# Xingskcs/Distributed-TensorFlow-Examples

Hardware: AMD Instinct MI355X
Metric: images/sec (whole node), MNIST CNN sync all-reduce (higher is better)
Workload: dtype bf16; 1 GPU; model=mnist_cnn (conv5x5x32-pool-conv5x5x64-pool-fc1024-dropout-fc10, 3274634 params), global_batch=1024, parallelism=dp1, per_gpu_batch=1024, optimizer=adam (TF1), hip_graph=True, steps_per_graph=4, join_deferred=True, distinct_gpus=1, grad_allreduce=none (1 rank), ranks_seen_by_comm=1

## Files before the change

csrc/kernels/imgconv12_fused.hip:

```cpp
#include "imgconv.h"
#include "imgconv1_common.h"

namespace dtfe {

namespace {

using namespace c1;

constexpr int WAVES = 13, THREADS = 64 * WAVES;
constexpr int CS = 32, KH = 5, KW = 5, LWP = 20, PS = 48, N2 = 64, NT = N2 / 16;
constexpr int K2 = KH * KW * CS, NK = K2 / 32, KP = K2 + 16;
constexpr int PH = HI / 2;
constexpr int LH = PH + KH - 1;
constexpr int QH = PH / 2, Q2 = QH * QH;
constexpr int P1N = PH * PH * NCH;
constexpr int P2N = Q2 * N2;
constexpr int W_EL = N2 * KP, IMG_EL = LH * LWP * PS;
constexpr int STAGE_B = P2N * 3, COPIES_B = 8 * CSZ * 2;
constexpr int UNION_B = COPIES_B > STAGE_B ? COPIES_B : STAGE_B;
constexpr int P_B = PRW * PWD * 2;
constexpr int LDS_B = W_EL * 2 + IMG_EL * 2 + UNION_B + P_B;
static_assert(W_EL * 2 == 104448 && IMG_EL * 2 == 34560 && STAGE_B == 9408 && COPIES_B == 20608 && P_B == 3072,
              "LDS regions");
static_assert(LDS_B == 162688 && LDS_B <= 160 * 1024, "LDS budget");
static_assert(K2 % 32 == 0 && PS >= CS + NCH / 2, "a pixel's pad bytes hold its 32 argmax bytes");
static_assert((PH * PH + 15) / 16 == WAVES, "one conv2 row tile per wave");

struct Conv12Args {
  ImgConvArgs c1;
  const bf16* w2;
  const float* b2;
  bf16* p2;
  uint8_t* a2;
};

template <int B, int E, typename F>
__device__ __forceinline__ void static_for(F&& f) {
  if constexpr (B < E) {
    f(std::integral_constant<int, B>{});
    static_for<B + 1, E>(f);
  }
}

__device__ __forceinline__ int row_window(int m) {
  const int t = m >> 4, quad = (m >> 2) & 3;
  const int w = t * 4 + (quad == 0 ? 0 : quad == 1 ? 2 : quad == 2 ? 3 : 1);
  return w < Q2 ? w : -1;
}

__global__ __launch_bounds__(THREADS) void conv12_fwd_kernel(Conv12Args A) {
  extern __shared__ __attribute__((aligned(16))) bf16 lds[];
  bf16* wl = lds;
  bf16* img = wl + W_EL;
  bf16* C = img + IMG_EL;
  bf16* sy = C;
  uint8_t* sa = reinterpret_cast<uint8_t*>(sy + P2N);
  bf16* P = C + UNION_B / 2;
  const ImgConvArgs& a = A.c1;
  const int tid = threadIdx.x, lane = tid & 63, wid = __builtin_amdgcn_readfirstlane(tid >> 6), g = lane >> 4;

  for (int i = tid; i < IMG_EL / 8; i += THREADS) reinterpret_cast<u32x4_t*>(img)[i] = u32x4_t{0u, 0u, 0u, 0u};
  for (int i = tid; i < PRW * PWD / 8; i += THREADS) reinterpret_cast<u32x4_t*>(P)[i] = u32x4_t{0u, 0u, 0u, 0u};

  const int64_t gstep = *a.g_counter;
  for (int z = 0; z < a.nz; ++z)
    for (long i = (long)blockIdx.x * THREADS + tid; i < a.zlen[z]; i += (long)gridDim.x * THREADS) a.zptr[z][i] = 0u;

  uint32_t px = 0u;
  int32_t lab = 0;
  auto fetch = [&](long bb) {
    const long r = (long)(hash_u32(a.g_seed, (uint64_t)gstep * a.B + bb) % (uint32_t)a.g_rows);
    if (tid < XCH) px = *reinterpret_cast<const uint32_t*>(a.g_src + r * (HI * HI) + tid * 4);
    if (tid == 0) lab = a.g_labels_src[r];
  };
  long b = blockIdx.x;
  if (b < a.B) fetch(b);

  {
    constexpr int kc_row = KP / 8, total = N2 * kc_row;
    static_assert(total <= 8 * THREADS, "one pass");
    u32x4_t v[8];
    int off[8];
#pragma unroll
    for (int u = 0; u < 8; ++u) {
      const int i = tid + u * THREADS;
      const int n = i / kc_row, k = (i - n * kc_row) * 8;
      off[u] = i < total ? n * KP + k : -1;
      v[u] = u32x4_t{0u, 0u, 0u, 0u};
      if (i < total && k < K2) v[u] = *reinterpret_cast<const u32x4_t*>(A.w2 + (long)n * K2 + k);
    }
#pragma unroll
    for (int u = 0; u < 8; ++u)
      if (off[u] >= 0) *reinterpret_cast<u32x4_t*>(wl + off[u]) = v[u];
  }

  bf16x8_t bw[2][2];
  float bias1[2];
  load_conv1_weights(a.w, a.bias, lane, g, bw, bias1);

  const bf16* wlane = wl + (lane & 15) * KP + 8 * g;
  float bias2[NT];
#pragma unroll
  for (int n = 0; n < NT; ++n) bias2[n] = A.b2 ? A.b2[n * 16 + (lane & 15)] : 0.f;
  const bf16* abase;
  {
    const int m = wid * 16 + (lane & 15), w = row_window(m), q = m & 3;
    const int oy = 2 * (w / QH) + (q >> 1), ox = 2 * (w % QH) + (q & 1);
    abase = img + (w >= 0 ? (oy * LWP + ox) * PS : 0) + 8 * g;
  }
  const int ppix = row_window(wid * 16 + g * 4);

  __syncthreads();
  for (; b < a.B; b += gridDim.x) {
    if (tid < XCH) {
      const u32x2_t v = px4_to_bf16(px);
      *reinterpret_cast<u32x2_t*>(const_cast<bf16*>(a.src) + b * (HI * HI) + tid * 4) = v;
      write_img(P, v);
    }
    if (tid == 0 && a.g_labels_dst) a.g_labels_dst[b] = lab;
    __syncthreads();
    if (b + gridDim.x < a.B) fetch(b + gridDim.x);
    build_copies8_by4(P, C);
    __syncthreads();

    for (int t = wid; t < 49; t += WAVES) {
      const int m = t * 16 + (lane & 15), q = m & 3, w = m >> 2;
      const int oy = 2 * (w / 14) + (q >> 1), ox = 2 * (w % 14) + (q & 1);
      const int s = ox & 7;
      const bf16* ab = C + s * CSZ + (ox - s) + oy * CWD;
      const bf16x8_t a0 = __builtin_bit_cast(bf16x8_t, ld16l(ab + g * CWD));
      const bf16x8_t a1 = __builtin_bit_cast(bf16x8_t, ld16l(ab + 4 * CWD));
      f32x4_t acc[2];
#pragma unroll
      for (int nt = 0; nt < 2; ++nt) {
        acc[nt] = __builtin_amdgcn_mfma_f32_16x16x32_bf16(a0, bw[nt][0], f32x4_t{0.f, 0.f, 0.f, 0.f}, 0, 0, 0);
        acc[nt] = __builtin_amdgcn_mfma_f32_16x16x32_bf16(a1, bw[nt][1], acc[nt], 0, 0, 0);
      }
      const int wq = t * 4 + g, py = wq / 14, pxx = wq - py * 14;
      bf16* pp = img + ((py + 2) * LWP + pxx + 2) * PS;
      uint8_t* pa = reinterpret_cast<uint8_t*>(pp + CS);
#pragma unroll
      for (int nt = 0; nt < 2; ++nt) {
        const f32x4_t v = acc[nt];
        int am = 0;
        float mx = v[0];
#pragma unroll
        for (int j = 1; j < 4; ++j) if (v[j] > mx) { mx = v[j]; am = j; }
        const int ch = nt * 16 + (lane & 15);
        pp[ch] = f2bf(apply_act(mx + bias1[nt], ACT_RELU));
        pa[ch] = (uint8_t)am;
      }
    }
    __syncthreads();

    {
      const long ob = b * (long)P1N;
      for (int i = tid; i < P1N / 8 + P1N / 16; i += THREADS) {
        const bool isv = i < P1N / 8;
        const int k = isv ? i : i - P1N / 8;
        const int pix = isv ? k >> 2 : k >> 1, py = pix / PH, pxx = pix - py * PH;
        const bf16* pp = img + ((py + 2) * LWP + pxx + 2) * PS;
        if (isv) {
          *reinterpret_cast<u32x4_t*>(a.y + ob + k * 8) = *reinterpret_cast<const u32x4_t*>(pp + (k & 3) * 8);
        } else {
          *reinterpret_cast<u32x4_t*>(a.argmax + ob + k * 16) =
              *reinterpret_cast<const u32x4_t*>(reinterpret_cast<const uint8_t*>(pp + CS) + (k & 1) * 16);
        }
      }
    }

    f32x4_t acc[NT];
#pragma unroll
    for (int n = 0; n < NT; ++n) acc[n] = f32x4_t{0.f, 0.f, 0.f, 0.f};
    constexpr int PF = 2;
    u32x4_t fa[PF + 1], fb[PF + 1][NT];
    auto fetch_frag = [&](auto sc) {
      constexpr int st = decltype(sc)::value;
      constexpr int k0 = 32 * st, tap = k0 / CS, cs = k0 - tap * CS;
      constexpr int toff = ((tap / KW) * LWP + (tap % KW)) * PS + cs;
      constexpr int buf = st % (PF + 1);
      fa[buf] = *reinterpret_cast<const u32x4_t*>(abase + toff);
#pragma unroll
      for (int n = 0; n < NT; ++n) fb[buf][n] = *reinterpret_cast<const u32x4_t*>(wlane + n * 16 * KP + k0);
    };
    static_for<0, PF>([&](auto sc) { fetch_frag(sc); });
    static_for<0, NK>([&](auto sc) {
      constexpr int st = decltype(sc)::value;
      if constexpr (st + PF < NK) fetch_frag(std::integral_constant<int, st + PF>{});
      constexpr int buf = st % (PF + 1);
#pragma unroll
      for (int n = 0; n < NT; ++n)
        acc[n] = __builtin_amdgcn_mfma_f32_16x16x32_bf16(__builtin_bit_cast(bf16x8_t, fa[buf]),
                                                         __builtin_bit_cast(bf16x8_t, fb[buf][n]), acc[n], 0, 0, 0);
      constexpr int nm = NT, nr = (st + PF < NK) ? 1 + NT : 0;
      static_for<0, nm>([&](auto ic) {
        constexpr int i = decltype(ic)::value, r0 = i * nr / nm, r1 = (i + 1) * nr / nm;
        if constexpr (r1 > r0) __builtin_amdgcn_sched_group_barrier(0x100, r1 - r0, 0);
        __builtin_amdgcn_sched_group_barrier(0x8, 1, 0);
      });
    });
    if (ppix >= 0) {
#pragma unroll
      for (int n = 0; n < NT; ++n) {
        const int col = n * 16 + (lane & 15);
        const f32x4_t v = acc[n];
        int am = 0;
        float mx = v[0];
#pragma unroll
        for (int j = 1; j < 4; ++j) if (v[j] > mx) { mx = v[j]; am = j; }
        sy[ppix * N2 + col] = f2bf(apply_act(mx + bias2[n], ACT_RELU));
        sa[ppix * N2 + col] = (uint8_t)am;
      }
    }
    __syncthreads();
    {
      constexpr int ny = P2N / 8, na = P2N / 16;
      const long pb = b * (long)P2N;
      for (int i = tid; i < ny + na; i += THREADS) {
        if (i < ny) {
          *reinterpret_cast<u32x4_t*>(A.p2 + pb + i * 8) = *reinterpret_cast<const u32x4_t*>(sy + i * 8);
        } else {
          const int k = i - ny;
          *reinterpret_cast<u32x4_t*>(A.a2 + pb + k * 16) = *reinterpret_cast<const u32x4_t*>(sa + k * 16);
        }
      }
    }
  }
  if (a.g_done && tid == 0) {
    const uint32_t prev = __hip_atomic_fetch_add(a.g_done, 1u, __ATOMIC_RELAXED, __HIP_MEMORY_SCOPE_AGENT);
    if (prev == gridDim.x - 1) {
      __hip_atomic_fetch_add((unsigned long long*)a.g_counter, 1ull, __ATOMIC_RELAXED, __HIP_MEMORY_SCOPE_AGENT);
      __hip_atomic_store(a.g_done, 0u, __ATOMIC_RELAXED, __HIP_MEMORY_SCOPE_AGENT);
    }
  }
}

}

bool launch_conv12_fused_fwd(const ImgConvArgs& a, const bf16* w2, const float* b2, bf16* p2, uint8_t* a2,
                             hipStream_t s) {
  if (a.B < 256 || a.SH != HI || a.SW != HI || a.CS != 1 || a.OH != HI || a.OW != HI || a.N != NCH || a.KH != 5 ||
      a.KW != 5 || a.stride != 1 || a.pad != 2)
    return false;
  if (!a.src || !a.pool || a.flip_taps || a.dil > 1 || a.relu_mask || a.act != ACT_RELU) return false;
  if (!a.g_src || !a.g_counter || !a.g_labels_src || !a.y || !a.argmax || !w2 || !p2 || !a2) return false;
  Conv12Args A{a, w2, b2, p2, a2};
  A.c1.diag = 0;
  const int grid = a.B < 256 ? a.B : 256;
  (void)hipFuncSetAttribute((const void*)conv12_fwd_kernel, hipFuncAttributeMaxDynamicSharedMemorySize, LDS_B);
  hipLaunchKernelGGL(conv12_fwd_kernel, dim3(grid), dim3(THREADS), LDS_B, s, A);
  return true;
}

}
```

csrc/kernels/imgconv1_common.h:

```cpp
#pragma once
#include "common.h"

#include <type_traits>

namespace dtfe {
namespace c1 {

constexpr int TH = 256;
constexpr int HI = 28;
constexpr int PWD = 48, PRW = 32;
constexpr int CWD = 40;
constexpr int CSZ = PRW * CWD + 8;
constexpr int NCH = 32;
constexpr int XCH = HI * HI / 4;

__device__ __forceinline__ u32x4_t ld16l(const bf16* p) { return *reinterpret_cast<const u32x4_t*>(p); }

template <int B, int E, typename F>
__device__ __forceinline__ void static_for_c1(F&& f) {
  if constexpr (B < E) {
    f(std::integral_constant<int, B>{});
    static_for_c1<B + 1, E>(f);
  }
}

__device__ __forceinline__ void load_img(const bf16* x, long b, u32x2_t& v) {
  if (threadIdx.x < XCH) v = *reinterpret_cast<const u32x2_t*>(x + b * (HI * HI) + threadIdx.x * 4);
}
__device__ __forceinline__ void write_img(bf16* P, const u32x2_t& v) {
  if (threadIdx.x < XCH) {
    const int r = threadIdx.x / 7, c = (threadIdx.x - r * 7) * 4;
    *reinterpret_cast<u32x2_t*>(P + (r + 2) * PWD + c + 4) = v;
  }
}

__device__ __forceinline__ u32x2_t px4_to_bf16(uint32_t px) {
  const float k = 1.f / 255.f;
  return u32x2_t{pack_bf16x2((float)(px & 0xffu) * k, (float)((px >> 8) & 0xffu) * k),
                 pack_bf16x2((float)((px >> 16) & 0xffu) * k, (float)(px >> 24) * k)};
}

__device__ __forceinline__ uint32_t shr16(uint32_t lo, uint32_t hi) {
  return (uint32_t)((((uint64_t)hi << 32) | lo) >> 16);
}
template <int S>
__device__ __forceinline__ void build_copies(const bf16* P, bf16* C) {
  constexpr int HALF = (S + 1) / 2;
  const int t = threadIdx.x & 127, r = t >> 2, c8 = (t & 3) * 8;
  const u32x4_t* src = reinterpret_cast<const u32x4_t*>(P + r * PWD + c8);
  uint32_t d[12];
#pragma unroll
  for (int j = 0; j < 3; ++j) {
    const u32x4_t v = src[j];
#pragma unroll
    for (int e = 0; e < 4; ++e) d[4 * j + e] = v[e];
  }
  auto emit = [&](auto sc) {
    constexpr int s = decltype(sc)::value;
    constexpr int e0 = s + 2;
    u32x4_t o;
#pragma unroll
    for (int j = 0; j < 4; ++j) o[j] = (e0 & 1) ? shr16(d[(e0 >> 1) + j], d[(e0 >> 1) + j + 1]) : d[(e0 >> 1) + j];
    *reinterpret_cast<u32x4_t*>(C + s * CSZ + r * CWD + c8) = o;
  };
  if (threadIdx.x < 128) {
    static_for_c1<0, HALF>(emit);
  } else {
    static_for_c1<HALF, S>(emit);
  }
}

__device__ __forceinline__ void build_copies8_by4(const bf16* P, bf16* C) {
  if (threadIdx.x >= 512) return;
  const int t = threadIdx.x & 127, r = t >> 2, c8 = (t & 3) * 8;
  const u32x4_t* src = reinterpret_cast<const u32x4_t*>(P + r * PWD + c8);
  uint32_t d[12];
#pragma unroll
  for (int j = 0; j < 3; ++j) {
    const u32x4_t v = src[j];
#pragma unroll
    for (int e = 0; e < 4; ++e) d[4 * j + e] = v[e];
  }
  auto emit = [&](auto sc) {
    constexpr int s = decltype(sc)::value;
    constexpr int e0 = s + 2;
    u32x4_t o;
#pragma unroll
    for (int j = 0; j < 4; ++j) o[j] = (e0 & 1) ? shr16(d[(e0 >> 1) + j], d[(e0 >> 1) + j + 1]) : d[(e0 >> 1) + j];
    *reinterpret_cast<u32x4_t*>(C + s * CSZ + r * CWD + c8) = o;
  };
  switch (threadIdx.x >> 7) {
    case 0: static_for_c1<0, 2>(emit); break;
    case 1: static_for_c1<2, 4>(emit); break;
    case 2: static_for_c1<4, 6>(emit); break;
    default: static_for_c1<6, 8>(emit); break;
  }
}

__device__ __forceinline__ void load_conv1_weights(const bf16* w, const float* bias, int lane, int g,
                                                   bf16x8_t (&bw)[2][2], float (&biasv)[2]) {
#pragma unroll
  for (int nt = 0; nt < 2; ++nt) {
    const int n = nt * 16 + (lane & 15);
    biasv[nt] = bias ? bias[n] : 0.f;
#pragma unroll
    for (int st = 0; st < 2; ++st) {
      const int kh = st == 0 ? g : 4;
      const bool rowok = st == 0 || g == 0;
      s16x8_t v;
#pragma unroll
      for (int j = 0; j < 8; ++j) v[j] = (short)((rowok && j < 5) ? w[n * 25 + kh * 5 + j] : 0);
      bw[nt][st] = __builtin_bit_cast(bf16x8_t, v);
    }
  }
}

}
}
```

Before: 5.609 million images/sec.

## Add producer waves that stage next image while conv2 runs on compute waves

Adds three producer waves beside the thirteen conv2 waves. While the compute waves run the conv2 MFMA loop, the producer waves store conv1 outputs to global memory, convert and stage the next image, and build its shifted copies, which removes two block-wide barriers per image from the critical path. The conv2 pooled output staging moves into padding chunks of the weight, copy and image LDS regions to free the union buffer. Conv1 tiles are batched three per wave with loads hoisted ahead of the MFMAs. The larger block and tighter LDS aliasing add complexity and a risk of register pressure.

```diff
diff --git a/csrc/kernels/imgconv12_fused.hip b/csrc/kernels/imgconv12_fused.hip
--- a/csrc/kernels/imgconv12_fused.hip
+++ b/csrc/kernels/imgconv12_fused.hip
@@ -7,7 +7,8 @@
 
 using namespace c1;
 
-constexpr int WAVES = 13, THREADS = 64 * WAVES;
+constexpr int CW = 13, SW = 3;
+constexpr int WAVES = CW + SW, THREADS = 64 * WAVES;
 constexpr int CS = 32, KH = 5, KW = 5, LWP = 20, PS = 48, N2 = 64, NT = N2 / 16;
 constexpr int K2 = KH * KW * CS, NK = K2 / 32, KP = K2 + 16;
 constexpr int PH = HI / 2;
@@ -17,14 +18,26 @@
 constexpr int P2N = Q2 * N2;
 constexpr int W_EL = N2 * KP, IMG_EL = LH * LWP * PS;
 constexpr int STAGE_B = P2N * 3, COPIES_B = 8 * CSZ * 2;
-constexpr int UNION_B = COPIES_B > STAGE_B ? COPIES_B : STAGE_B;
 constexpr int P_B = PRW * PWD * 2;
-constexpr int LDS_B = W_EL * 2 + IMG_EL * 2 + UNION_B + P_B;
+constexpr int LDS_B = W_EL * 2 + IMG_EL * 2 + COPIES_B + P_B;
 static_assert(W_EL * 2 == 104448 && IMG_EL * 2 == 34560 && STAGE_B == 9408 && COPIES_B == 20608 && P_B == 3072,
               "LDS regions");
 static_assert(LDS_B == 162688 && LDS_B <= 160 * 1024, "LDS budget");
 static_assert(K2 % 32 == 0 && PS >= CS + NCH / 2, "a pixel's pad bytes hold its 32 argmax bytes");
-static_assert((PH * PH + 15) / 16 == WAVES, "one conv2 row tile per wave");
+static_assert((PH * PH + 15) / 16 == CW, "one conv2 row tile per wave");
+static_assert(3 * WAVES < 49 && 49 <= 3 * WAVES + 1, "conv1: 3 tiles per wave and tile 48 for wave 0");
+
+constexpr int PIXB = PS * 2;
+constexpr int ST_C = 8 * PRW, ST_W = 2 * N2, ST_I = STAGE_B / 16 - ST_C - ST_W;
+constexpr int ST_IROW = (LWP - (PH + KW - 1)) * PIXB / 16;
+static_assert(CWD - 32 == 8 && CSZ == PRW * CWD + 8 && KP - K2 == 16 && PIXB % 16 == 0, "pad chunks");
+static_assert(ST_I > 0 && ST_I <= LH * ST_IROW, "the padding holds the staging");
+__device__ __forceinline__ int stage_off(int c) {
+  if (c < ST_C) return W_EL * 2 + IMG_EL * 2 + c * (CWD * 2) + (c / PRW) * 16 + 64;
+  if (c < ST_C + ST_W) return ((c - ST_C) >> 1) * (KP * 2) + K2 * 2 + ((c - ST_C) & 1) * 16;
+  const int i = c - ST_C - ST_W, row = i / ST_IROW;
+  return W_EL * 2 + (row * LWP + PH + KW - 1) * PIXB + (i - row * ST_IROW) * 16;
+}
 
 struct Conv12Args {
   ImgConvArgs c1;
@@ -48,42 +61,95 @@
   return w < Q2 ? w : -1;
 }
 
+__device__ __forceinline__ int opaque(int v) {
+  asm volatile("" : "+v"(v));
+  return v;
+}
+
 __global__ __launch_bounds__(THREADS) void conv12_fwd_kernel(Conv12Args A) {
+  constexpr int NP = (((PRW + SW - 1) / SW) * 7 + 63) / 64;
+  static_assert(((PRW + SW - 1) / SW) * 4 <= 64, "a lane per (row, 16-B column chunk) of the wave's copy rows");
   extern __shared__ __attribute__((aligned(16))) bf16 lds[];
   bf16* wl = lds;
   bf16* img = wl + W_EL;
   bf16* C = img + IMG_EL;
-  bf16* sy = C;
-  uint8_t* sa = reinterpret_cast<uint8_t*>(sy + P2N);
-  bf16* P = C + UNION_B / 2;
+  bf16* P = C + COPIES_B / 2;
+  uint8_t* stg = reinterpret_cast<uint8_t*>(lds);
   const ImgConvArgs& a = A.c1;
   const int tid = threadIdx.x, lane = tid & 63, wid = __builtin_amdgcn_readfirstlane(tid >> 6), g = lane >> 4;
 
   for (int i = tid; i < IMG_EL / 8; i += THREADS) reinterpret_cast<u32x4_t*>(img)[i] = u32x4_t{0u, 0u, 0u, 0u};
-  for (int i = tid; i < PRW * PWD / 8; i += THREADS) reinterpret_cast<u32x4_t*>(P)[i] = u32x4_t{0u, 0u, 0u, 0u};
 
   const int64_t gstep = *a.g_counter;
   for (int z = 0; z < a.nz; ++z)
     for (long i = (long)blockIdx.x * THREADS + tid; i < a.zlen[z]; i += (long)gridDim.x * THREADS) a.zptr[z][i] = 0u;
 
-  uint32_t px = 0u;
+  const int sw = wid - CW;
+  const bool producer = sw >= 0;
+  const int r0 = sw * PRW / SW, r1 = (sw + 1) * PRW / SW;
+  const int c0 = 7 * (r0 > 2 ? r0 - 2 : 0), nc = 7 * (r1 - 2 < HI ? r1 - 2 : HI) - c0;
+  uint32_t px[NP];
   int32_t lab = 0;
+#pragma unroll
+  for (int u = 0; u < NP; ++u) px[u] = 0u;
   auto fetch = [&](long bb) {
     const long r = (long)(hash_u32(a.g_seed, (uint64_t)gstep * a.B + bb) % (uint32_t)a.g_rows);
-    if (tid < XCH) px = *reinterpret_cast<const uint32_t*>(a.g_src + r * (HI * HI) + tid * 4);
-    if (tid == 0) lab = a.g_labels_src[r];
+    const int ln = opaque(lane);
+#pragma unroll
+    for (int u = 0; u < NP; ++u)
+      if (ln + 64 * u < nc) px[u] = *reinterpret_cast<const uint32_t*>(a.g_src + r * (HI * HI) + (c0 + ln + 64 * u) * 4);
+    if (sw == 0 && lane == 0) lab = a.g_labels_src[r];
+  };
+  auto stage = [&](long bb) {
+    const int ln = opaque(lane);
+#pragma unroll
+    for (int u = 0; u < NP; ++u)
+      if (ln + 64 * u < nc) {
+        const int id = c0 + ln + 64 * u, r = id / 7, c = (id - r * 7) * 4;
+        const u32x2_t v = px4_to_bf16(px[u]);
+        *reinterpret_cast<u32x2_t*>(const_cast<bf16*>(a.src) + bb * (HI * HI) + id * 4) = v;
+        *reinterpret_cast<u32x2_t*>(P + (r + 2) * PWD + c + 4) = v;
+      }
+    if (sw == 0 && lane == 0 && a.g_labels_dst) a.g_labels_dst[bb] = lab;
+    __builtin_amdgcn_fence(__ATOMIC_RELEASE, "wavefront");
+    __builtin_amdgcn_wave_barrier();
+    const int r = r0 + (ln >> 2), c8 = (ln & 3) * 8;
+    if (r < r1) {
+      const u32x4_t* src = reinterpret_cast<const u32x4_t*>(P + r * PWD + c8);
+      uint32_t d[12];
+#pragma unroll
+      for (int j = 0; j < 3; ++j) {
+        const u32x4_t v = src[j];
+#pragma unroll
+        for (int e = 0; e < 4; ++e) d[4 * j + e] = v[e];
+      }
+      static_for<0, 8>([&](auto sc) {
+        constexpr int s = decltype(sc)::value;
+        constexpr int e0 = s + 2;
+        u32x4_t o;
+#pragma unroll
+        for (int j = 0; j < 4; ++j) o[j] = (e0 & 1) ? shr16(d[(e0 >> 1) + j], d[(e0 >> 1) + j + 1]) : d[(e0 >> 1) + j];
+        *reinterpret_cast<u32x4_t*>(C + s * CSZ + r * CWD + c8) = o;
+      });
+    }
   };
   long b = blockIdx.x;
-  if (b < a.B) fetch(b);
-
-  {
+  if (producer) {
+    if (b < a.B) fetch(b);
+    for (int k = lane; k < (r1 - r0) * (PWD / 8); k += 64)
+      reinterpret_cast<u32x4_t*>(P + r0 * PWD)[k] = u32x4_t{0u, 0u, 0u, 0u};
+    if (b < a.B) {
+      stage(b);
+      if (b + gridDim.x < a.B) fetch(b + gridDim.x);
+    }
+  } else {
     constexpr int kc_row = KP / 8, total = N2 * kc_row;
-    static_assert(total <= 8 * THREADS, "one pass");
+    static_assert(total <= 8 * 64 * CW, "one pass");
     u32x4_t v[8];
     int off[8];
 #pragma unroll
     for (int u = 0; u < 8; ++u) {
-      const int i = tid + u * THREADS;
+      const int i = tid + u * 64 * CW;
       const int n = i / kc_row, k = (i - n * kc_row) * 8;
       off[u] = i < total ? n * KP + k : -1;
       v[u] = u32x4_t{0u, 0u, 0u, 0u};
@@ -112,50 +178,16 @@
 
   __syncthreads();
   for (; b < a.B; b += gridDim.x) {
-    if (tid < XCH) {
-      const u32x2_t v = px4_to_bf16(px);
-      *reinterpret_cast<u32x2_t*>(const_cast<bf16*>(a.src) + b * (HI * HI) + tid * 4) = v;
-      write_img(P, v);
-    }
-    if (tid == 0 && a.g_labels_dst) a.g_labels_dst[b] = lab;
-    __syncthreads();
-    if (b + gridDim.x < a.B) fetch(b + gridDim.x);
-    build_copies8_by4(P, C);
-    __syncthreads();
-
-    for (int t = wid; t < 49; t += WAVES) {
-      const int m = t * 16 + (lane & 15), q = m & 3, w = m >> 2;
-      const int oy = 2 * (w / 14) + (q >> 1), ox = 2 * (w % 14) + (q & 1);
-      const int s = ox & 7;
-      const bf16* ab = C + s * CSZ + (ox - s) + oy * CWD;
-      const bf16x8_t a0 = __builtin_bit_cast(bf16x8_t, ld16l(ab + g * CWD));
-      const bf16x8_t a1 = __builtin_bit_cast(bf16x8_t, ld16l(ab + 4 * CWD));
-      f32x4_t acc[2];
-#pragma unroll
-      for (int nt = 0; nt < 2; ++nt) {
-        acc[nt] = __builtin_amdgcn_mfma_f32_16x16x32_bf16(a0, bw[nt][0], f32x4_t{0.f, 0.f, 0.f, 0.f}, 0, 0, 0);
-        acc[nt] = __builtin_amdgcn_mfma_f32_16x16x32_bf16(a1, bw[nt][1], acc[nt], 0, 0, 0);
-      }
-      const int wq = t * 4 + g, py = wq / 14, pxx = wq - py * 14;
-      bf16* pp = img + ((py + 2) * LWP + pxx + 2) * PS;
-      uint8_t* pa = reinterpret_cast<uint8_t*>(pp + CS);
-#pragma unroll
-      for (int nt = 0; nt < 2; ++nt) {
-        const f32x4_t v = acc[nt];
-        int am = 0;
-        float mx = v[0];
-#pragma unroll
-        for (int j = 1; j < 4; ++j) if (v[j] > mx) { mx = v[j]; am = j; }
-        const int ch = nt * 16 + (lane & 15);
-        pp[ch] = f2bf(apply_act(mx + bias1[nt], ACT_RELU));
-        pa[ch] = (uint8_t)am;
-      }
-    }
-    __syncthreads();
-
-    {
+    const bool more = b + gridDim.x < a.B;
+    auto stage_next = [&]() {
+      if (more) {
+        stage(b + gridDim.x);
+        if (b + 2 * (long)gridDim.x < a.B) fetch(b + 2 * (long)gridDim.x);
+      }
+    };
+    auto store_p1a1 = [&]() {
       const long ob = b * (long)P1N;
-      for (int i = tid; i < P1N / 8 + P1N / 16; i += THREADS) {
+      for (int i = opaque(tid) - 64 * CW; i < P1N / 8 + P1N / 16; i += 64 * SW) {
         const bool isv = i < P1N / 8;
         const int k = isv ? i : i - P1N / 8;
         const int pix = isv ? k >> 2 : k >> 1, py = pix / PH, pxx = pix - py * PH;
@@ -167,49 +199,99 @@
               *reinterpret_cast<const u32x4_t*>(reinterpret_cast<const uint8_t*>(pp + CS) + (k & 1) * 16);
         }
       }
-    }
+    };
+
+    {
+      constexpr int TPW = (49 + WAVES - 1) / WAVES;
+      bf16x8_t fa0[TPW], fa1[TPW];
+      f32x4_t acc[TPW][2];
+      static_for<0, TPW>([&](auto jc) {
+        constexpr int j = decltype(jc)::value;
+        const int t = j < TPW - 1 ? wid + j * WAVES : 48;
+        const int m = t * 16 + (lane & 15), q = m & 3, w = m >> 2;
+        const int oy = 2 * (w / 14) + (q >> 1), ox = 2 * (w % 14) + (q & 1);
+        const int s = ox & 7;
+        const bf16* ab = C + s * CSZ + (ox - s) + oy * CWD;
+        fa0[j] = __builtin_bit_cast(bf16x8_t, ld16l(ab + g * CWD));
+        fa1[j] = __builtin_bit_cast(bf16x8_t, ld16l(ab + 4 * CWD));
+      });
+      static_for<0, TPW>([&](auto jc) {
+        constexpr int j = decltype(jc)::value;
+#pragma unroll
+        for (int nt = 0; nt < 2; ++nt) {
+          acc[j][nt] = __builtin_amdgcn_mfma_f32_16x16x32_bf16(fa0[j], bw[nt][0], f32x4_t{0.f, 0.f, 0.f, 0.f}, 0, 0, 0);
+          acc[j][nt] = __builtin_amdgcn_mfma_f32_16x16x32_bf16(fa1[j], bw[nt][1], acc[j][nt], 0, 0, 0);
+        }
+      });
+      static_for<0, TPW>([&](auto jc) {
+        constexpr int j = decltype(jc)::value;
+        if (j < TPW - 1 || wid == 0) {
+          const int t = j < TPW - 1 ? wid + j * WAVES : 48;
+          const int wq = t * 4 + g, py = wq / 14, pxx = wq - py * 14;
+          bf16* pp = img + ((py + 2) * LWP + pxx + 2) * PS;
+          uint8_t* pa = reinterpret_cast<uint8_t*>(pp + CS);
+#pragma unroll
+          for (int nt = 0; nt < 2; ++nt) {
+            const f32x4_t v = acc[j][nt];
+            int am = 0;
+            float mx = v[0];
+#pragma unroll
+            for (int e = 1; e < 4; ++e) if (v[e] > mx) { mx = v[e]; am = e; }
+            const int ch = nt * 16 + (lane & 15);
+            pp[ch] = f2bf(apply_act(mx + bias1[nt], ACT_RELU));
+            pa[ch] = (uint8_t)am;
+          }
+        }
+      });
+    }
+    __syncthreads();
 
     f32x4_t acc[NT];
 #pragma unroll
     for (int n = 0; n < NT; ++n) acc[n] = f32x4_t{0.f, 0.f, 0.f, 0.f};
-    constexpr int PF = 2;
-    u32x4_t fa[PF + 1], fb[PF + 1][NT];
-    auto fetch_frag = [&](auto sc) {
-      constexpr int st = decltype(sc)::value;
-      constexpr int k0 = 32 * st, tap = k0 / CS, cs = k0 - tap * CS;
-      constexpr int toff = ((tap / KW) * LWP + (tap % KW)) * PS + cs;
-      constexpr int buf = st % (PF + 1);
-      fa[buf] = *reinterpret_cast<const u32x4_t*>(abase + toff);
-#pragma unroll
-      for (int n = 0; n < NT; ++n) fb[buf][n] = *reinterpret_cast<const u32x4_t*>(wlane + n * 16 * KP + k0);
-    };
-    static_for<0, PF>([&](auto sc) { fetch_frag(sc); });
-    static_for<0, NK>([&](auto sc) {
-      constexpr int st = decltype(sc)::value;
-      if constexpr (st + PF < NK) fetch_frag(std::integral_constant<int, st + PF>{});
-      constexpr int buf = st % (PF + 1);
-#pragma unroll
-      for (int n = 0; n < NT; ++n)
-        acc[n] = __builtin_amdgcn_mfma_f32_16x16x32_bf16(__builtin_bit_cast(bf16x8_t, fa[buf]),
-                                                         __builtin_bit_cast(bf16x8_t, fb[buf][n]), acc[n], 0, 0, 0);
-      constexpr int nm = NT, nr = (st + PF < NK) ? 1 + NT : 0;
-      static_for<0, nm>([&](auto ic) {
-        constexpr int i = decltype(ic)::value, r0 = i * nr / nm, r1 = (i + 1) * nr / nm;
-        if constexpr (r1 > r0) __builtin_amdgcn_sched_group_barrier(0x100, r1 - r0, 0);
-        __builtin_amdgcn_sched_group_barrier(0x8, 1, 0);
-      });
-    });
+    if (wid < CW) {
+      constexpr int PF = 2;
+      u32x4_t fa[PF + 1], fb[PF + 1][NT];
+      auto fetch_frag = [&](auto sc) {
+        constexpr int st = decltype(sc)::value;
+        constexpr int k0 = 32 * st, tap = k0 / CS, cs = k0 - tap * CS;
+        constexpr int toff = ((tap / KW) * LWP + (tap % KW)) * PS + cs;
+        constexpr int buf = st % (PF + 1);
+        fa[buf] = *reinterpret_cast<const u32x4_t*>(abase + toff);
+#pragma unroll
+        for (int n = 0; n < NT; ++n) fb[buf][n] = *reinterpret_cast<const u32x4_t*>(wlane + n * 16 * KP + k0);
+      };
+      static_for<0, PF>([&](auto sc) { fetch_frag(sc); });
+      static_for<0, NK>([&](auto sc) {
+        constexpr int st = decltype(sc)::value;
+        if constexpr (st + PF < NK) fetch_frag(std::integral_constant<int, st + PF>{});
+        constexpr int buf = st % (PF + 1);
+#pragma unroll
+        for (int n = 0; n < NT; ++n)
+          acc[n] = __builtin_amdgcn_mfma_f32_16x16x32_bf16(__builtin_bit_cast(bf16x8_t, fa[buf]),
+                                                           __builtin_bit_cast(bf16x8_t, fb[buf][n]), acc[n], 0, 0, 0);
+        constexpr int nm = NT, nr = (st + PF < NK) ? 1 + NT : 0;
+        static_for<0, nm>([&](auto ic) {
+          constexpr int i = decltype(ic)::value, r0 = i * nr / nm, r1 = (i + 1) * nr / nm;
+          if constexpr (r1 > r0) __builtin_amdgcn_sched_group_barrier(0x100, r1 - r0, 0);
+          __builtin_amdgcn_sched_group_barrier(0x8, 1, 0);
+        });
+      });
+    } else {
+      store_p1a1();
+      stage_next();
+    }
     if (ppix >= 0) {
 #pragma unroll
       for (int n = 0; n < NT; ++n) {
-        const int col = n * 16 + (lane & 15);
+        const int col = n * 16 + (lane & 15), e = ppix * N2 + col;
         const f32x4_t v = acc[n];
         int am = 0;
         float mx = v[0];
 #pragma unroll
         for (int j = 1; j < 4; ++j) if (v[j] > mx) { mx = v[j]; am = j; }
-        sy[ppix * N2 + col] = f2bf(apply_act(mx + bias2[n], ACT_RELU));
-        sa[ppix * N2 + col] = (uint8_t)am;
+        *reinterpret_cast<bf16*>(stg + stage_off(e >> 3) + (e & 7) * 2) = f2bf(apply_act(mx + bias2[n], ACT_RELU));
+        stg[stage_off(P2N / 8 + (e >> 4)) + (e & 15)] = (uint8_t)am;
       }
     }
     __syncthreads();
@@ -217,11 +299,11 @@
       constexpr int ny = P2N / 8, na = P2N / 16;
       const long pb = b * (long)P2N;
       for (int i = tid; i < ny + na; i += THREADS) {
+        const u32x4_t v = *reinterpret_cast<const u32x4_t*>(stg + stage_off(i));
         if (i < ny) {
-          *reinterpret_cast<u32x4_t*>(A.p2 + pb + i * 8) = *reinterpret_cast<const u32x4_t*>(sy + i * 8);
+          *reinterpret_cast<u32x4_t*>(A.p2 + pb + i * 8) = v;
         } else {
-          const int k = i - ny;
-          *reinterpret_cast<u32x4_t*>(A.a2 + pb + k * 16) = *reinterpret_cast<const u32x4_t*>(sa + k * 16);
+          *reinterpret_cast<u32x4_t*>(A.a2 + pb + (i - ny) * 16) = v;
         }
       }
     }
diff --git a/csrc/kernels/imgconv1_common.h b/csrc/kernels/imgconv1_common.h
--- a/csrc/kernels/imgconv1_common.h
+++ b/csrc/kernels/imgconv1_common.h
@@ -70,33 +70,6 @@
   }
 }
 
-__device__ __forceinline__ void build_copies8_by4(const bf16* P, bf16* C) {
-  if (threadIdx.x >= 512) return;
-  const int t = threadIdx.x & 127, r = t >> 2, c8 = (t & 3) * 8;
-  const u32x4_t* src = reinterpret_cast<const u32x4_t*>(P + r * PWD + c8);
-  uint32_t d[12];
-#pragma unroll
-  for (int j = 0; j < 3; ++j) {
-    const u32x4_t v = src[j];
-#pragma unroll
-    for (int e = 0; e < 4; ++e) d[4 * j + e] = v[e];
-  }
-  auto emit = [&](auto sc) {
-    constexpr int s = decltype(sc)::value;
-    constexpr int e0 = s + 2;
-    u32x4_t o;
-#pragma unroll
-    for (int j = 0; j < 4; ++j) o[j] = (e0 & 1) ? shr16(d[(e0 >> 1) + j], d[(e0 >> 1) + j + 1]) : d[(e0 >> 1) + j];
-    *reinterpret_cast<u32x4_t*>(C + s * CSZ + r * CWD + c8) = o;
-  };
-  switch (threadIdx.x >> 7) {
-    case 0: static_for_c1<0, 2>(emit); break;
-    case 1: static_for_c1<2, 4>(emit); break;
-    case 2: static_for_c1<4, 6>(emit); break;
-    default: static_for_c1<6, 8>(emit); break;
-  }
-}
-
 __device__ __forceinline__ void load_conv1_weights(const bf16* w, const float* bias, int lane, int g,
                                                    bf16x8_t (&bw)[2][2], float (&biasv)[2]) {
 #pragma unroll
```

Result: faster. 5.721 million images/sec, median of 6 (+2.0%).
